# foxcroftjn/polars-strsim

Hardware: AMD Instinct MI355X
Metric: M string-pairs/s, levenshtein, 100 M rows (+ achieved HBM GB/s in roofline) (higher is better)
Workload: dtype u8/u32 bit-parallel, f64 epilogue

## Files before the change

polars-strsim_amd/csrc/strsim_lane_core.h:

```cpp
#pragma once
#include <stdint.h>
#include <type_traits>

#if defined(__HIPCC__)
#define STRSIM_HD __host__ __device__ __forceinline__
#else
#define STRSIM_HD inline
#endif

namespace strsim {

enum Measure : int { LEVENSHTEIN = 0, JARO = 1, JARO_WINKLER = 2, JACCARD = 3, SORENSEN_DICE = 4 };


#ifndef STRSIM_COLS_PER_TEST
#define STRSIM_COLS_PER_TEST 2
#endif
constexpr int COLS_PER_TEST = STRSIM_COLS_PER_TEST;

STRSIM_HD uint32_t lane_byte(const uint32_t (&w)[8], int j) { return (w[j >> 2] >> ((j & 3) * 8)) & 0xFFu; }

STRSIM_HD uint32_t low_ones(uint32_t k) { return k >= 32u ? 0xFFFFFFFFu : ((1u << k) - 1u); }

template <int G, int NG, typename F>
// ... 105 lines not shown
            r[4 * h + 1] = perm_b32(t2, t0, 0x07060302u);
            r[4 * h + 2] = perm_b32(t3, t1, 0x05040100u);
            r[4 * h + 3] = perm_b32(t3, t1, 0x07060302u);
        }
    }
#pragma unroll
    for (int e = 0; e < 8; e += 2) {
        const uint32_t a = r[e], b = r[e + 1];
        r[e] = bitop3<0xCA>(0x55555555u, a, twice(b));
        r[e + 1] = bitop3<0xCA>(0x55555555u, a >> 1, b);
    }
#pragma unroll
    for (int q = 0; q < 4; ++q) {
        const int e = (q & 1) | ((q & 2) << 1);
        const uint32_t a = r[e], b = r[e + 2];
        r[e] = bitop3<0xCA>(0x33333333u, a, b << 2);
        r[e + 2] = bitop3<0xCA>(0x33333333u, a >> 2, b);
    }
#pragma unroll
    for (int e = 0; e < 4; ++e) {
        const uint32_t a = r[e], b = r[e + 4];
        if (e < NP) P[e < NP ? e : 0] = bitop3<0xCA>(0x0F0F0F0Fu, a, b << 4);
        if (e + 4 < NP) P[e + 4 < NP ? e + 4 : 0] = bitop3<0xCA>(0x0F0F0F0Fu, a >> 4, b);
    }
}

template <int NP>
STRSIM_HD uint32_t eq_mask(const uint32_t (&P)[NP], uint32_t valid, uint32_t w, int byte)
{
    uint32_t acc = valid;
#pragma unroll
    for (int k = 0; k < NP; ++k) acc = bitop3<0x90>(acc, P[k], bit_fill(w, 8 * byte + k));
    return acc;
}

STRSIM_HD int planes_needed(uint32_t vary) { return (vary & 0x40u) ? 7 : ((vary & 0x20u) ? 6 : 5); }

STRSIM_HD uint32_t window_vary(const uint32_t (&wa)[8], const uint32_t (&wb)[8], uint32_t &any)
{
    uint32_t o = bitop3<0xFE>(wa[0], wa[1], wa[2]), n = bitop3<0x80>(wa[0], wa[1], wa[2]);
    o = bitop3<0xFE>(o, wa[3], wa[4]); n = bitop3<0x80>(n, wa[3], wa[4]);
    o = bitop3<0xFE>(o, wa[5], wa[6]); n = bitop3<0x80>(n, wa[5], wa[6]);
    o = bitop3<0xFE>(o, wa[7], wb[0]); n = bitop3<0x80>(n, wa[7], wb[0]);
    o = bitop3<0xFE>(o, wb[1], wb[2]); n = bitop3<0x80>(n, wb[1], wb[2]);
    o = bitop3<0xFE>(o, wb[3], wb[4]); n = bitop3<0x80>(n, wb[3], wb[4]);
    o = bitop3<0xFE>(o, wb[5], wb[6]); n = bitop3<0x80>(n, wb[5], wb[6]);
    o |= wb[7]; n &= wb[7];
    uint32_t o8 = o | (o >> 16); o8 |= o8 >> 8;
    uint32_t n8 = n & (n >> 16); n8 &= n8 >> 8;
    any = o8 & 0xFFu;
    return (o8 ^ n8) & 0xFFu;
}

template <int NP>
STRSIM_HD uint32_t lev_myers32_snap(const uint32_t (&wt)[8], uint32_t lt, uint32_t tmin, uint32_t tmax, const uint32_t (&P)[NP],
                                    uint32_t lp)
{
    uint32_t Pv = 0xFFFFFFFFu, Mv = 0u;
#pragma unroll
    for (int g = 0; g < 32 / COLS_PER_TEST; ++g) {
        if ((uint32_t)(COLS_PER_TEST * g) >= tmax) break;
        auto column = [&](int j) {
            const uint32_t Eq = eq_mask<NP>(P, 0xFFFFFFFFu, wt[j >> 2], j & 3);
            const uint32_t D0 = bitop3<0xBE>((Eq & Pv) + Pv, Pv, Eq) | Mv;
            const uint32_t nHP = bitop3<0x0E>(Mv, D0, Pv);
            const uint32_t nX = twice(nHP);
            const uint32_t HN2 = twice(D0 & Pv);
            Pv = bitop3<0xF2>(HN2, D0, nX);
            Mv = bitop3<0x50>(D0, D0, nX);
        };
        if ((uint32_t)(COLS_PER_TEST * (g + 1)) >= tmin) {
#pragma unroll
            for (int jj = 0; jj < COLS_PER_TEST; ++jj)
                if ((uint32_t)(COLS_PER_TEST * g + jj) < lt) column(COLS_PER_TEST * g + jj);
        } else {
#pragma unroll
            for (int jj = 0; jj < COLS_PER_TEST; ++jj) column(COLS_PER_TEST * g + jj);
        }
    }
    const uint32_t rows = low_ones(lp);
    return lt + popc32(Pv & rows) - popc32(Mv & rows);
}

STRSIM_HD uint32_t common_prefix4(uint32_t a0, uint32_t la, uint32_t b0, uint32_t lb)
{
    const uint32_t x = a0 ^ b0;
    uint32_t p = 4u;
    if (x & 0x000000FFu) p = 0u;
    else if (x & 0x0000FF00u) p = 1u;
    else if (x & 0x00FF0000u) p = 2u;
    else if (x & 0xFF000000u) p = 3u;
    if (p > la) p = la;
    if (p > lb) p = lb;
    return p;
}

STRSIM_HD double epilogue_levenshtein(uint64_t dist, uint64_t la, uint64_t lb)
{
    const uint64_t den = la > lb ? la : lb;
    return 1.0 - ((double)dist / (double)den);
}

STRSIM_HD double epilogue_jaro(uint64_t m, uint64_t t, uint64_t la, uint64_t lb)
{
    if (m == 0) return 0.0;
    const double dm = (double)m;
    return (dm / (double)la + dm / (double)lb + (double)(m - t / 2) / dm) / 3.0;
}

STRSIM_HD double epilogue_jaro_winkler(double jaro, uint32_t prefix)
{
    if (jaro > 0.7) {
        const double pl = (double)prefix;
        return jaro + (pl * 0.1 * (1.0 - jaro));
    }
    return jaro;
}

STRSIM_HD double epilogue_jaccard(uint64_t isect, uint64_t la, uint64_t lb)
{
    return (double)isect / (double)(la + lb - isect);
}

STRSIM_HD double epilogue_sorensen_dice(uint64_t isect, uint64_t la, uint64_t lb)
{
    return 2.0 * (double)isect / (double)(la + lb);
}
// ... 93 lines not shown
```

polars-strsim_amd/csrc/strsim_lane_stage.h:

```cpp
#pragma once

#ifndef STRSIM_STAGE_ROWS
#define STRSIM_STAGE_ROWS 512
#endif
#ifndef STRSIM_STAGE_CAP
#define STRSIM_STAGE_CAP 10240
#endif
#ifndef STRSIM_STAGE_CAP_LONG
#define STRSIM_STAGE_CAP_LONG 15104
#endif
#ifndef STRSIM_STAGE_CAP_LUT
#define STRSIM_STAGE_CAP_LUT 8960
#endif
#ifndef STRSIM_STAGE_WAVES_PER_EU
#define STRSIM_STAGE_WAVES_PER_EU 5
#endif
#ifndef STRSIM_STAGE_BUCKET_SHIFT
#define STRSIM_STAGE_BUCKET_SHIFT 1
#endif

#ifndef STRSIM_STAGE_LUT
#define STRSIM_STAGE_LUT 0x26
#endif
#ifndef STRSIM_JARO_KEEP_EQ_FILLS
#define STRSIM_JARO_KEEP_EQ_FILLS 1
#endif
#ifndef STRSIM_STAGE_LONG_TEXT_MAX
#define STRSIM_STAGE_LONG_TEXT_MAX 32
#endif
#ifndef STRSIM_STAGE_RANGE_MAX
#define STRSIM_STAGE_RANGE_MAX 64
#endif
#ifndef STRSIM_STAGE_RANGE_DIV
#define STRSIM_STAGE_RANGE_DIV 4
#endif
#ifndef STRSIM_STAGE_RANGE_MIN_BLOCKS
#define STRSIM_STAGE_RANGE_MIN_BLOCKS 2
#endif

#if defined(STRSIM_LAB) && defined(STRSIM_STAGE_STAMPS)
__device__ unsigned long long g_stage_stamps[16384][16];
#define STAGE_STAMP(cat) do { __builtin_amdgcn_sched_barrier(0); const unsigned long long t_ = __builtin_amdgcn_s_memtime(); \
                              __builtin_amdgcn_sched_barrier(0); st_acc[cat] += t_ - st_last; st_last = t_; } while (0)
#else
#define STAGE_STAMP(cat) do { } while (0)
#endif

#ifndef STRSIM_STAGE_THREADS
#define STRSIM_STAGE_THREADS 256
#endif
constexpr int STAGE_BLOCK = STRSIM_STAGE_THREADS;
constexpr int STAGE_WAVES = STAGE_BLOCK / 64;
constexpr int STAGE_ROWS = STRSIM_STAGE_ROWS;
constexpr int STAGE_RPT = STAGE_ROWS / STAGE_BLOCK;
constexpr int STAGE_NR = STAGE_ROWS / 64;
constexpr int STAGE_RPW = STAGE_NR / STAGE_WAVES;
template <int MEASURE> constexpr bool stage_uses_lut() { return ((STRSIM_STAGE_LUT >> MEASURE) & 1) != 0; }

template <bool TABLES, bool LONG = false> struct StageGeom {
    static_assert(!(TABLES && LONG), "the long-row geometry has no match-mask tables");
    static constexpr int CAP = LONG ? STRSIM_STAGE_CAP_LONG : (TABLES ? STRSIM_STAGE_CAP_LUT : STRSIM_STAGE_CAP);
    static constexpr int COL = CAP + 96;
    static constexpr int DMA_ITERS = (CAP + 48 + 16 * STAGE_BLOCK - 1) / (16 * STAGE_BLOCK);
    static_assert(CAP % 16 == 0 && 2 * COL + 64 + 16 <= 65536, "staging area: whole wave-instructions, 16-bit LDS offsets");
};
constexpr int STAGE_BSH = STRSIM_STAGE_BUCKET_SHIFT;
constexpr int STAGE_NBK = (32 >> STAGE_BSH) + 1;
static_assert(STAGE_RPT >= 1 && STAGE_RPT <= 4 && STAGE_RPW >= 1, "STAGE_ROWS is 256, 512 or 1024");
static_assert(STAGE_NBK <= 32, "the bucket scan runs on 32 lanes");

#define STRSIM_LDS_ADDR(p) ((uint32_t)(uintptr_t)((__attribute__((address_space(3))) void *)(p)))

__device__ __forceinline__ void lds_dma_b128(const void *gbase, uint32_t goff, uint32_t lds_dst)
{
    uint32_t keep;
    asm volatile("s_mov_b32 %0, m0\n\ts_mov_b32 m0, %3\n\ts_nop 0\n\tglobal_load_lds_dwordx4 %1, %2\n\ts_mov_b32 m0, %0"
                 : "=&s"(keep)
                 : "v"(goff), "s"(gbase), "s"(lds_dst)
                 : "memory");
}
__device__ __forceinline__ void lds_dma_b32(const void *gbase, uint32_t goff, uint32_t lds_dst)
{
    uint32_t keep;
    asm volatile("s_mov_b32 %0, m0\n\ts_mov_b32 m0, %3\n\ts_nop 0\n\tglobal_load_lds_dword %1, %2\n\ts_mov_b32 m0, %0"
                 : "=&s"(keep)
                 : "v"(goff), "s"(gbase), "s"(lds_dst)
                 : "memory");
}

__device__ __forceinline__ uint32_t load_invariant(const uint32_t *p)
{
    return *reinterpret_cast<const __attribute__((address_space(4))) uint32_t *>(reinterpret_cast<uintptr_t>(p));
}

constexpr uint32_t STAGE_DEAD = 1u << 31;

#if defined(STRSIM_LAB) && defined(STRSIM_STAGE_STRIP)
__device__ const uint16_t *g_strip_ptr;
__global__ __launch_bounds__(256) void k_strip_oracle(const uint32_t *__restrict__ offA, const uint8_t *__restrict__ valA, const uint32_t *__restrict__ offB,
                                                      const uint8_t *__restrict__ valB, uint64_t n, uint16_t *__restrict__ out)
{
    const uint64_t r = (uint64_t)blockIdx.x * 256u + threadIdx.x;
    if (r >= n) return;
    const uint32_t a0 = offA[r], la = offA[r + 1] - a0, b0 = offB[r], lb = offB[r + 1] - b0;
    const uint32_t m = la < lb ? la : lb, cap = (uint32_t)STRSIM_STAGE_STRIP;
    uint32_t p = 0, s = 0;
    while (p < m && p < cap && valA[a0 + p] == valB[b0 + p]) ++p;
    while (s < m - p && s < cap && valA[a0 + la - 1u - s] == valB[b0 + lb - 1u - s]) ++s;
    if (p + s > 63u) s = 63u - p;
    out[r] = (uint16_t)(p | (s << 8));
}
#define STRSIM_STRIP_ON 1
#else
#define STRSIM_STRIP_ON 0
#endif

__device__ __forceinline__ void stage_window(const uint8_t *base, uint32_t at, uint32_t (&w)[8], uint32_t lds_bytes = 0u, uint32_t who = 0u)
{
    typedef uint32_t u32x4_a4 __attribute__((ext_vector_type(4), aligned(4)));
    (void)lds_bytes; (void)who;
    if (who == 1u) STRSIM_CHECK_RANGE(K_STAGE, 40, ~0ull, (at & ~3u) + 36u, 0, lds_bytes);
    if (who == 2u) STRSIM_CHECK_RANGE(K_LIT, 40, ~0ull, (at & ~3u) + 36u, 0, lds_bytes);
    const uint8_t *q = base + (at & ~3u);
    const u32x4_a4 lo = *reinterpret_cast<const u32x4_a4 *>(q);
    const u32x4_a4 hi = *reinterpret_cast<const u32x4_a4 *>(q + 16);
    const uint32_t top = *reinterpret_cast<const uint32_t *>(q + 32);
    const uint32_t sh = at & 3u;
    w[0] = __builtin_amdgcn_alignbyte(lo.y, lo.x, sh); w[1] = __builtin_amdgcn_alignbyte(lo.z, lo.y, sh);
    w[2] = __builtin_amdgcn_alignbyte(lo.w, lo.z, sh); w[3] = __builtin_amdgcn_alignbyte(hi.x, lo.w, sh);
    w[4] = __builtin_amdgcn_alignbyte(hi.y, hi.x, sh); w[5] = __builtin_amdgcn_alignbyte(hi.z, hi.y, sh);
    w[6] = __builtin_amdgcn_alignbyte(hi.w, hi.z, sh); w[7] = __builtin_amdgcn_alignbyte(top, hi.w, sh);
}

__device__ __forceinline__ uint32_t scan32_inclusive(uint32_t x)
{
    x += (uint32_t)__builtin_amdgcn_update_dpp(0, (int)x, 0x111, 0xF, 0xF, true);
    x += (uint32_t)__builtin_amdgcn_update_dpp(0, (int)x, 0x112, 0xF, 0xF, true);
    x += (uint32_t)__builtin_amdgcn_update_dpp(0, (int)x, 0x114, 0xF, 0xF, true);
    x += (uint32_t)__builtin_amdgcn_update_dpp(0, (int)x, 0x118, 0xF, 0xF, true);
    x += (uint32_t)__builtin_amdgcn_update_dpp(0, (int)x, 0x142, 0xA, 0xF, true);
    return x;
}

template <int NP, bool USE_LUT>
__device__ __forceinline__ uint32_t stage_lev_code(const EqLut &lut, const uint32_t (&wa)[8], uint32_t la, const uint32_t (&wb)[8],
                                                   uint32_t lb, uint32_t tmin, uint32_t tmax, uint32_t stripped = 0u)
{
    uint32_t P[NP];
    build_planes<NP>(wb, P);
    EqLut t = lut;
    if (USE_LUT) lut_build<NP>(t, P, 0xFFFFFFFFu);
    const bool live = la != 0u && lb != 0u;
    const uint32_t la1 = live ? la : 1u, lb1 = live ? lb : 1u;
    const uint32_t dist = USE_LUT ? lev_myers32_lut<NP>(t, wa, la1, tmin, tmax, P, lb1) : lev_myers32_snap<NP>(wa, la1, tmin, tmax, P, lb1);
    uint32_t code = dist * (uint32_t)QTAB_N + (la1 > lb1 ? la1 : lb1);
    if (!live) code = (la == 0u && lb == 0u) ? 1u : (uint32_t)QTAB_N + 1u;
#if STRSIM_STRIP_ON
    const uint32_t longer = la > lb ? la : lb;
    code = (live ? dist : longer) * (uint32_t)QTAB_N + (longer + stripped);
#endif
    return code;
}

template <int NP, bool USE_LUT>
__device__ __forceinline__ unsigned long long stage_all_ints(const EqLut &lut, const uint32_t (&wa)[8], uint32_t la,
                                                             const uint32_t (&wb)[8], uint32_t lb, uint32_t tmin, uint32_t tmax)
{
    uint32_t P[NP];
    build_planes<NP>(wb, P);
    const bool live = la != 0u && lb != 0u;
    const uint32_t la1 = live ? la : 1u, lb1 = live ? lb : 1u;
    uint32_t dist, m, t, isect;
    if (USE_LUT) {
        EqLut tb = lut;
        lut_build<NP>(tb, P, 0xFFFFFFFFu);
        lane_cores32_lut<NP, true, true, true>(tb, wa, la1, tmin, tmax, lb1, P, dist, m, t, isect);
    } else {
        lane_cores32<NP, true, true, true>(wa, la1, tmin, tmax, lb1, P, dist, m, t, isect);
    }
    const uint32_t pre = common_prefix4(wa[0], la1, wb[0], lb1);
    const uint32_t lo = dist | (m << 6) | (t << 12) | (isect << 18) | (pre << 24) | (la << 27);
    return (unsigned long long)lo | ((unsigned long long)(la >> 5) << 32) | ((unsigned long long)lb << 33);
}

__device__ __forceinline__ void stage_all_epilogues(unsigned long long pk, double qa, double qb, double qc, double qd, double (&r)[5])
{
    const uint32_t lo = (uint32_t)pk, hi = (uint32_t)(pk >> 32);
    const uint32_t m = (lo >> 6) & 63u, isect = (lo >> 18) & 63u, pre = (lo >> 24) & 7u;
    const uint32_t la = ((lo >> 27) & 31u) | ((hi & 1u) << 5), lb = (hi >> 1) & 63u;
    if (la == 0u || lb == 0u) {
        const double v = (la == 0u && lb == 0u) ? 1.0 : 0.0;
#pragma unroll
        for (int q = 0; q < 5; ++q) r[q] = v;
        return;
    }
    r[LEVENSHTEIN] = 1.0 - qd;
    const double j = m == 0u ? 0.0 : div3_exact(qa + qb + qc);
    r[JARO] = j;
    r[JARO_WINKLER] = epilogue_jaro_winkler(j, pre);
    r[JACCARD] = epilogue_jaccard(isect, la, lb);
    r[SORENSEN_DICE] = epilogue_sorensen_dice(isect, la, lb);
}

template <int MEASURE, int NP, bool USE_LUT>
__device__ __forceinline__ uint32_t stage_ints(const EqLut &lut, const uint32_t (&wa)[8], uint32_t la, const uint32_t (&wb)[8],
                                               uint32_t lb, uint32_t tmin, uint32_t tmax)
{
    uint32_t P[NP];
    build_planes<NP>(wb, P);
    const bool live = la != 0u && lb != 0u;
    const uint32_t la1 = live ? la : 1u, lb1 = live ? lb : 1u;
    uint32_t dist, m, t, isect;
    EqLut tb = lut;
    if (USE_LUT) lut_build<NP>(tb, P, 0xFFFFFFFFu);
    if (MEASURE == JARO || MEASURE == JARO_WINKLER) {
        if (USE_LUT) lane_cores32_lut<NP, false, true, false>(tb, wa, la1, tmin, tmax, lb1, P, dist, m, t, isect);
        else lane_cores32<NP, false, true, false, STRSIM_JARO_KEEP_EQ_FILLS != 0>(wa, la1, tmin, tmax, lb1, P, dist, m, t, isect);
        const uint32_t pre = MEASURE == JARO_WINKLER ? common_prefix4(wa[0], la1, wb[0], lb1) : 0u;
        return m | (t << 6) | (la << 12) | (lb << 18) | (pre << 24);
    }
    if (USE_LUT) lane_cores32_lut<NP, false, false, true>(tb, wa, la1, tmin, tmax, lb1, P, dist, m, t, isect);
    else lane_cores32<NP, false, false, true>(wa, la1, tmin, tmax, lb1, P, dist, m, t, isect);
    return isect | (la << 6) | (lb << 12);
}

template <int MEASURE>
__device__ __forceinline__ double stage_epilogue(uint32_t pk, double qa, double qb, double qc)
{
    if (MEASURE == JARO || MEASURE == JARO_WINKLER) {
        const uint32_t m = pk & 63u, la = (pk >> 12) & 63u, lb = (pk >> 18) & 63u, pre = (pk >> 24) & 7u;
        if (la == 0u || lb == 0u) return (la == 0u && lb == 0u) ? 1.0 : 0.0;
        const double j = m == 0u ? 0.0 : div3_exact(qa + qb + qc);
        return MEASURE == JARO_WINKLER ? epilogue_jaro_winkler(j, pre) : j;
    }
    const uint32_t isect = pk & 63u, la = (pk >> 6) & 63u, lb = (pk >> 12) & 63u;
    if (la == 0u || lb == 0u) return (la == 0u && lb == 0u) ? 1.0 : 0.0;
    return MEASURE == JACCARD ? epilogue_jaccard(isect, la, lb) : epilogue_sorensen_dice(isect, la, lb);
}

template <int MEASURE, bool LUT>
__device__ __forceinline__ void stage_compute(const EqLut &lut, const uint32_t (&wt)[8], const uint32_t (&wp)[8], uint32_t meta,
                                              uint32_t last, uint16_t *s_code, uint32_t *s_word, double *s_val)
{
    bool fast = (meta & STAGE_DEAD) == 0u;
#if STRSIM_STRIP_ON
    const uint32_t lt = meta & 0x3Fu, lp = (meta >> 8) & 0x3Fu, idx = (meta >> 16) & 0x1FFu, stripped = (meta >> 25) & 0x3Fu;
#else
    const uint32_t lt = meta & 0x3Fu, lp = (meta >> 8) & 0x3Fu, idx = (meta >> 16) & 0x7FFu, stripped = 0u;
#endif
    uint32_t any;
    const uint32_t vary = window_vary(wt, wp, any);
    if (any & 0x80u) fast = false;
    if (__ballot(fast) == 0ull) return;
    const uint32_t la = fast ? lt : 0u, lb = fast ? lp : 0u;
    static_assert((1 << STAGE_BSH) % COLS_PER_TEST == 0, "a bucket's upper bound is a whole number of column groups");
    const uint32_t ltl = (uint32_t)__builtin_amdgcn_readlane((int)lt, (int)last);
    const uint32_t tmax = (((ltl ? ltl : 1u) - 1u) | ((1u << STAGE_BSH) - 1u)) + 1u;
    const bool wide = __ballot(fast && (vary & 0x60u)) != 0ull;
    const uint32_t lt0 = uniform(lt);
    const uint32_t tmin = (((lt0 ? lt0 : 1u) - 1u) & ~((1u << STAGE_BSH) - 1u)) + 1u;
    if (MEASURE == LEVENSHTEIN) {
        uint32_t code;
        if (wide) code = stage_lev_code<7, LUT>(lut, wt, la, wp, lb, tmin, tmax, stripped);
        else code = stage_lev_code<5, LUT>(lut, wt, la, wp, lb, tmin, tmax, stripped);
        if (fast) STRSIM_CHECK_INDEX(K_STAGE, 42, ~0ull, idx, STAGE_ROWS);
        if (fast) s_code[idx] = (uint16_t)code;
    } else if (MEASURE == ALL_MEASURES) {
        unsigned long long pk;
        if (wide) pk = stage_all_ints<7, LUT>(lut, wt, la, wp, lb, tmin, tmax);
        else pk = stage_all_ints<5, LUT>(lut, wt, la, wp, lb, tmin, tmax);
        if (fast) STRSIM_CHECK_INDEX(K_STAGE, 43, ~0ull, idx, STAGE_ROWS);
        if (fast) reinterpret_cast<unsigned long long *>(s_val)[idx] = pk;
    } else {
        uint32_t pk;
        if (wide) pk = stage_ints<MEASURE, 7, LUT>(lut, wt, la, wp, lb, tmin, tmax);
        else pk = stage_ints<MEASURE, 5, LUT>(lut, wt, la, wp, lb, tmin, tmax);
        if (fast) STRSIM_CHECK_INDEX(K_STAGE, 44, ~0ull, idx, STAGE_ROWS);
        if (fast) s_word[idx] = pk;
    }
}

template <int MEASURE, bool LUT, bool LONG = false>
__device__ __forceinline__ void
lane_stage_body(const uint32_t *__restrict__ offA, const uint8_t *__restrict__ valA, uint64_t rowsA,
             const uint32_t *__restrict__ offB, const uint8_t *__restrict__ valB, uint64_t rowsB, OutPtrs outs,
             uint64_t n, unsigned long long *__restrict__ slowmask, DevStatus *__restrict__ status,
             const double *__restrict__ qtab, uint32_t *__restrict__ sched, DevStatus *__restrict__ publish, uint32_t ticket)
{
    constexpr bool LEV = MEASURE == LEVENSHTEIN;
    constexpr bool ALL = MEASURE == ALL_MEASURES;
    constexpr int B = STAGE_ROWS, RPT = STAGE_RPT, NBK = STAGE_NBK;
    constexpr int STAGE_CAP = StageGeom<LUT, LONG>::CAP, STAGE_COL = StageGeom<LUT, LONG>::COL;
    constexpr int STAGE_DMA_ITERS = StageGeom<LUT, LONG>::DMA_ITERS;
    constexpr uint32_t COLB = STAGE_COL, LIT = 2u * STAGE_COL;
    static_assert(!LUT || (B <= 128 * STAGE_WAVES && LUT_WAVE_BYTES == 3072), "descriptor slices: 128 rows behind each wave's tables");
    __shared__ __attribute__((aligned(4096))) uint8_t s_lut[LUT ? 4096 * STAGE_WAVES : 16];
    __shared__ uint2 s_desc_own[LUT ? 1 : B];
    __shared__ __attribute__((aligned(4096))) uint8_t s_bytes[2 * STAGE_COL + 64 + 16];
    auto desc_at = [&](uint32_t p) -> uint2 * {
        if (LUT) return reinterpret_cast<uint2 *>(s_lut + ((p >> 7) << 12) + LUT_WAVE_BYTES + ((p & 127u) << 3));
        return s_desc_own + p;
    };
    __shared__ __attribute__((aligned(16))) uint32_t s_off[2][B + 4];
    __shared__ uint32_t s_cnt[32];
    __shared__ uint32_t s_left;
    __shared__ uint32_t s_sched[2];
    __shared__ uint16_t s_code[LEV ? B : 1];
    __shared__ uint32_t s_word[(!LEV && !ALL) ? B : 1];
    __shared__ double s_val[ALL ? B : 1];

    const uint32_t tid = threadIdx.x, lane = lane_id(), wv = tid >> 6;
    if (blockIdx.x == 0u && tid < (uint32_t)(sizeof(DevStatus) / sizeof(uint32_t))) reinterpret_cast<uint32_t *>(status)[tid] = 0u;
    if (tid < 32u) s_cnt[tid] = 0u;
    if (tid == 0u) s_left = 0u;
#pragma unroll
    for (int q = 0; q < RPT; ++q) {
        const uint32_t i = (uint32_t)q * STAGE_BLOCK + tid;
        if (LEV) s_code[i] = 0xFFFFu;
        else if (ALL) reinterpret_cast<unsigned long long *>(&s_val[i])[0] = ~0ull;
        else s_word[i] = 0xFFFFFFFFu;
    }

    const uint32_t totalA = load_invariant(offA + rowsA), totalB = load_invariant(offB + rowsB);
#if STRSIM_BOUNDS_ON
    const uint32_t firstA = load_invariant(offA), firstB = load_invariant(offB);
#endif
    const bool bcastA = rowsA == 1, bcastB = rowsB == 1;
    const uint32_t litA0 = bcastA ? load_invariant(offA) : 0u, litB0 = bcastB ? load_invariant(offB) : 0u;
    const uint32_t litAlen = bcastA ? totalA - litA0 : 0u, litBlen = bcastB ? totalB - litB0 : 0u;
    if (wv == 0u) {
        auto literal_window = [&](const uint8_t *val, uint32_t at, uint32_t total, uint32_t len, uint32_t *dst) {
            uint32_t w[8];
            load_window32(val, at, total, w);
            const uint32_t rep = (w[0] & 0xFFu) * 0x01010101u;
#pragma unroll
            for (int q = 0; q < 8; ++q) {
                const uint32_t v = len > 4u * q ? (len - 4u * q < 4u ? len - 4u * q : 4u) : 0u;
                const uint32_t keep = v >= 4u ? 0xFFFFFFFFu : ((1u << (8u * v)) - 1u);
                dst[q] = (w[q] & keep) | (rep & ~keep);
            }
        };
        if (bcastA) literal_window(valA, litA0, totalA, litAlen, reinterpret_cast<uint32_t *>(s_bytes + LIT));
        if (bcastB) literal_window(valB, litB0, totalB, litBlen, reinterpret_cast<uint32_t *>(s_bytes + LIT + 32u));
    }
    const uint64_t nchunks = (n + 63u) >> 6;
    const uint32_t nchunks32 = (uint32_t)nchunks;
    auto grab = [&](uint32_t seen, uint32_t &lo, uint32_t &sz) {
        const uint32_t left = nchunks32 > seen ? nchunks32 - seen : 0u;
        uint32_t want = (uint32_t)STRSIM_STAGE_RANGE_MAX;
        if (left < (uint32_t)(STRSIM_STAGE_RANGE_MAX * STRSIM_STAGE_RANGE_DIV) * gridDim.x) want = left / ((uint32_t)STRSIM_STAGE_RANGE_DIV * gridDim.x);
        sz = want < (uint32_t)(STRSIM_STAGE_RANGE_MIN_BLOCKS * (B / 64)) ? (uint32_t)(STRSIM_STAGE_RANGE_MIN_BLOCKS * (B / 64)) : want;
        lo = __hip_atomic_fetch_add(&sched[0], sz, __ATOMIC_RELAXED, __HIP_MEMORY_SCOPE_AGENT);
    };
    uint32_t grab_lo = 0u, grab_sz = 0u;
    if (tid == 0u) {
        grab(0u, grab_lo, grab_sz);
        s_sched[0] = grab_lo;
        s_sched[1] = grab_sz;
    }
    lds_barrier();
    uint64_t row_end;
    uint64_t row0;
    {
        const uint64_t lo = uniform(s_sched[0]), hi = lo + uniform(s_sched[1]);
        row0 = lo * 64u < n ? lo * 64u : n;
        row_end = hi * 64u < n ? hi * 64u : n;
    }
// ... 84 lines not shown
            if (JARO_LIKE) { pin(t1[q]); pin(t2[q]); }
            if (ALL) pin(t3[q]);
        }
#pragma unroll
        for (int q = 0; q < RPT; ++q) {
            const uint32_t i = (uint32_t)q * STAGE_BLOCK + tid;
            if ((uint32_t)q * STAGE_BLOCK < rows) {
                bool undone;
                double v = 0.0, v5[5];
                if (ALL) {
                    undone = pk[q] == ~0ull;
                    if (!undone) stage_all_epilogues(pk[q], t0[q], t1[q], t2[q], t3[q], v5);
                } else if (LEV) {
                    undone = (uint32_t)pk[q] == 0xFFFFu;
                    v = 1.0 - t0[q];
                } else {
                    undone = (uint32_t)pk[q] == 0xFFFFFFFFu;
                    if (!undone) v = stage_epilogue<M1>((uint32_t)pk[q], t0[q], t1[q], t2[q]);
                }
                const bool valid = i < rows;
                const unsigned long long left = __ballot(undone && valid);
                if (valid) STRSIM_CHECK_INDEX(K_STAGE, 10, r0 + i, r0 + i, n);
                if (lane == 0u && valid) STRSIM_CHECK_INDEX(K_STAGE, 11, r0 + i, (r0 >> 6) + (i >> 6), nchunks);
                if (valid && !undone) {
                    if (ALL) {
#pragma unroll
                        for (int o = 0; o < 5; ++o) outs.p[o][r0 + i] = v5[o];
                    } else {
                        outs.p[0][r0 + i] = v;
                    }
                }
                if (lane == 0u && valid) {
                    maskb[i >> 6] = left;
                    if (publish && left) atomicAdd(&s_left, (uint32_t)__builtin_popcountll(left));
                }
            }
        }
    };

#if defined(STRSIM_LAB) && defined(STRSIM_STAGE_STAMPS)
    unsigned long long st_acc[10] = {0, 0, 0, 0, 0, 0, 0, 0, 0, 0};
    const unsigned long long st_t0 = __builtin_amdgcn_s_memtime(), st_r0 = __builtin_amdgcn_s_memrealtime();
    unsigned long long st_last = st_t0;
#endif
    while (row0 < row_end) {
        if (grab_pending) {
            if (tid == 0u) {
                s_sched[0] = grab_lo;
                s_sched[1] = grab_sz;
            }
            grab_pending = false;
        }
        if (prev_rows) store_block(prev_row0, prev_rows);
        STAGE_STAMP(1);
        const uint32_t avail = (uint32_t)(row_end - row0 < (uint64_t)B ? row_end - row0 : (uint64_t)B);
        const uint32_t baseA = bcastA ? litA0 : uniform(s_off[0][0]), baseB = bcastB ? litB0 : uniform(s_off[1][0]);
        const uint32_t misA = (uint32_t)(reinterpret_cast<uintptr_t>(valA + baseA) & 15u);
        const uint32_t misB = (uint32_t)(reinterpret_cast<uintptr_t>(valB + baseB) & 15u);
        uint32_t rows;
        {
            const uint32_t e = (lane + 1u) * 64u < avail ? (lane + 1u) * 64u : avail;
            const bool exists = lane * 64u < avail && lane < (uint32_t)(B / 64);
            const uint32_t endA = bcastA ? baseA : s_off[0][exists ? e : 0u], endB = bcastB ? baseB : s_off[1][exists ? e : 0u];
            const bool fits = exists && endA - baseA + misA <= (uint32_t)STAGE_CAP && endB - baseB + misB <= (uint32_t)STAGE_CAP;
            const unsigned long long okm = __ballot(fits);
            uint32_t k = (uint32_t)__builtin_ctzll(~okm);
            if (k == 0u) k = 1u;
            rows = uniform(k * 64u < avail ? k * 64u : avail);
        }
        const uint32_t endA = bcastA ? baseA : uniform(s_off[0][rows]), endB = bcastB ? baseB : uniform(s_off[1][rows]);
        const uint32_t spanA = endA - baseA + misA, spanB = endB - baseB + misB;
        const uint32_t stagedA = bcastA ? 0u : (((spanA < (uint32_t)STAGE_CAP ? spanA : (uint32_t)STAGE_CAP) + 15u) & ~15u);
        const uint32_t stagedB = bcastB ? 0u : (((spanB < (uint32_t)STAGE_CAP ? spanB : (uint32_t)STAGE_CAP) + 15u) & ~15u);
        const uint32_t leftA = totalA - baseA + misA, leftB = totalB - baseB + misB;
        const uint32_t chunksA = bcastA ? 0u : ((stagedA + 32u < leftA ? stagedA + 32u : leftA) + 15u) >> 4;
        const uint32_t chunksB = bcastB ? 0u : ((stagedB + 32u < leftB ? stagedB + 32u : leftB) + 15u) >> 4;
        if (tid < 2u) STRSIM_CHECK_RANGE(K_STAGE, 20, row0, (chunksA << 4) + tid * 16u + 16u, 0, COLB);
        else if (tid < 4u) STRSIM_CHECK_RANGE(K_STAGE, 21, row0, COLB + (chunksB << 4) + (tid - 2u) * 16u + 16u, 0, sizeof(s_bytes));
        if (tid < 2u) *reinterpret_cast<uint4 *>(s_bytes + (chunksA << 4) + tid * 16u) = make_uint4(0u, 0u, 0u, 0u);
        else if (tid < 4u) *reinterpret_cast<uint4 *>(s_bytes + COLB + (chunksB << 4) + (tid - 2u) * 16u) = make_uint4(0u, 0u, 0u, 0u);
        {
            const uint8_t *__restrict__ const gA = valA + baseA - misA, *__restrict__ const gB = valB + baseB - misB;
#pragma unroll
            for (int it = 0; it < STAGE_DMA_ITERS; ++it) {
                if (tid + (uint32_t)it * STAGE_BLOCK < chunksA) {
                    STRSIM_CHECK_COLUMN(K_STAGE, 22, row0, gA + 16 * it * STAGE_BLOCK + tid16, 16, valA, firstA, totalA);
                    STRSIM_CHECK_RANGE(K_STAGE, 23, row0, 16u * ((uint32_t)it * STAGE_BLOCK + tid) + 16u, 0, COLB);
                    lds_dma_b128(gA + 16 * it * STAGE_BLOCK, tid16, ldsBytes + 16u * ((uint32_t)it * STAGE_BLOCK + wvu * 64u));
                }
                if (tid + (uint32_t)it * STAGE_BLOCK < chunksB) {
                    STRSIM_CHECK_COLUMN(K_STAGE, 24, row0, gB + 16 * it * STAGE_BLOCK + tid16, 16, valB, firstB, totalB);
                    STRSIM_CHECK_RANGE(K_STAGE, 25, row0, COLB + 16u * ((uint32_t)it * STAGE_BLOCK + tid) + 16u, 0, sizeof(s_bytes));
                    lds_dma_b128(gB + 16 * it * STAGE_BLOCK, tid16, ldsBytes + COLB + 16u * ((uint32_t)it * STAGE_BLOCK + wvu * 64u));
                }
            }
        }
        STAGE_STAMP(0);
        uint32_t skey[RPT], srank[RPT], sd0[RPT], sd1[RPT];
        {
#pragma unroll
            for (int q = 0; q < RPT; ++q) {
                const uint32_t i = (uint32_t)RPT * tid + (uint32_t)q;
                STRSIM_CHECK_INDEX(K_STAGE, 30, row0, i + 1u, B + 4);
                const bool have = i < rows;
                const uint32_t a0 = bcastA ? 0u : s_off[0][i] - baseA, b0 = bcastB ? 0u : s_off[1][i] - baseB;
                const uint32_t la8 = bcastA ? litAlen : s_off[0][i + 1u] - s_off[0][i];
                const uint32_t lb8 = bcastB ? litBlen : s_off[1][i + 1u] - s_off[1][i];
                const bool stA = bcastA || misA + a0 + la8 <= stagedA, stB = bcastB || misB + b0 + lb8 <= stagedB;
                bool mine = have && la8 <= 32u && lb8 <= 32u && stA && stB;
                if (LONG && STRSIM_STAGE_LONG_TEXT_MAX < 32 && !bcastA && !bcastB) mine = mine && (la8 < lb8 ? la8 : lb8) <= (uint32_t)STRSIM_STAGE_LONG_TEXT_MAX;
                const uint32_t wa = bcastA ? LIT : misA + a0, wb = bcastB ? LIT + 32u : COLB + misB + b0;
                const bool swap = !bcastA && !bcastB && la8 > lb8;
#if STRSIM_STRIP_ON
                uint32_t sp = 0u, ss = 0u;
                if (LEV && !bcastA && !bcastB && have) {
                    const uint32_t ps = g_strip_ptr[row0 + i];
                    sp = ps & 0xFFu; ss = ps >> 8;
                }
                const uint32_t lt = (swap ? lb8 : la8) - sp - ss, lp = (swap ? la8 : lb8) - sp - ss;
                const uint32_t key = mine ? (((lt ? lt : 1u) - 1u) >> STAGE_BSH) : (uint32_t)(NBK - 1);
                skey[q] = key;
                srank[q] = atomicAdd(&s_cnt[key], 1u);
                sd0[q] = mine ? (swap ? ((wb + sp) | ((wa + sp) << 16)) : ((wa + sp) | ((wb + sp) << 16))) : 0u;
                sd1[q] = mine ? (lt | (lp << 8) | (i << 16) | ((sp + ss) << 25)) : STAGE_DEAD;
#else
                const uint32_t lt = swap ? lb8 : la8, lp = swap ? la8 : lb8;
                const uint32_t key = mine ? (((lt ? lt : 1u) - 1u) >> STAGE_BSH) : (uint32_t)(NBK - 1);
                skey[q] = key;
                srank[q] = atomicAdd(&s_cnt[key], 1u);
                sd0[q] = mine ? (swap ? (wb | (wa << 16)) : (wa | (wb << 16))) : 0u;
                sd1[q] = mine ? (lt | (lp << 8) | (i << 16)) : STAGE_DEAD;
#endif
            }
        }
        STAGE_STAMP(2);
        lds_barrier();
        STAGE_STAMP(3);
        uint32_t nmine;
        {
            const uint32_t c = s_cnt[lane & 31u];
            const uint32_t exc = scan32_inclusive(c) - c;
#pragma unroll
            for (int q = 0; q < RPT; ++q) {
                const uint32_t base = __shfl(exc, skey[q], 32);
                const uint32_t p = base + srank[q];
                STRSIM_CHECK_INDEX(K_STAGE, 31, row0, p, B);
                *desc_at(p) = make_uint2(sd0[q], sd1[q]);
            }
            nmine = uniform(__shfl(exc, NBK - 1, 32));
        }
        STAGE_STAMP(4);
        asm volatile("s_waitcnt vmcnt(0)" ::: "memory");
        if (!bcastA && leftA < (chunksA << 4) && tid == ((chunksA - 1u) & (uint32_t)(STAGE_BLOCK - 1)))
            for (uint32_t b = leftA; b < (chunksA << 4); ++b) { STRSIM_CHECK_INDEX(K_STAGE, 32, row0, b, COLB); s_bytes[b] = 0; }
        if (!bcastB && leftB < (chunksB << 4) && tid == ((chunksB - 1u) & (uint32_t)(STAGE_BLOCK - 1)))
            for (uint32_t b = leftB; b < (chunksB << 4); ++b) { STRSIM_CHECK_INDEX(K_STAGE, 33, row0, COLB + b, sizeof(s_bytes)); s_bytes[COLB + b] = 0; }
        lds_barrier();
        STAGE_STAMP(5);
        if (tid < 32u) s_cnt[tid] = 0u;
        uint64_t next_row0 = row0 + rows;
        if (next_row0 >= row_end) {
            const uint64_t lo = uniform(s_sched[0]), hi = lo + uniform(s_sched[1]);
            next_row0 = lo * 64u < n ? lo * 64u : n;
            row_end = hi * 64u < n ? hi * 64u : n;
            if (tid == 0u) grab((uint32_t)lo, grab_lo, grab_sz);
            grab_pending = true;
        }
        if (next_row0 < row_end) dma_offsets(next_row0);
        STAGE_STAMP(6);
        __builtin_amdgcn_s_setprio(0);
        {
            const uint32_t nrounds = (nmine + 63u) >> 6;
#pragma unroll 1
            for (int k = 0; k < STAGE_RPW; ++k) {
                const uint32_t t = (uint32_t)(k >> 1) * (2u * STAGE_WAVES) + ((k & 1) ? (uint32_t)(2 * STAGE_WAVES - 1) - wv : wv);
                if (t >= nrounds) continue;
                const uint32_t hi = nmine - 64u * t;
                const uint32_t first = hi >= 64u ? hi - 64u : 0u;
                const uint32_t in_round = hi - first;
                __builtin_amdgcn_s_setprio(1);
                STRSIM_CHECK_INDEX(K_STAGE, 41, row0, first + lane, B);
                const uint2 d = *desc_at(first + lane);
                uint32_t wt[8], wp[8];
                stage_window(s_bytes, d.x & 0xFFFFu, wt, (uint32_t)sizeof(s_bytes), STRSIM_BOUNDS_ON ? 1u : 0u);
                stage_window(s_bytes, d.x >> 16, wp, (uint32_t)sizeof(s_bytes), STRSIM_BOUNDS_ON ? 1u : 0u);
    #if defined(STRSIM_LAB) && defined(STRSIM_STAGE_STAMPS)
                asm volatile("s_waitcnt lgkmcnt(0)" ::: "memory");
    #endif
                STAGE_STAMP(7);
                __builtin_amdgcn_s_setprio(0);
                stage_compute<MEASURE, LUT>(lut, wt, wp, lane < in_round ? d.y : STAGE_DEAD, in_round - 1u, s_code, s_word, s_val);
                STAGE_STAMP(8);
            }
        }
        __builtin_amdgcn_s_setprio(1);
        asm volatile("s_waitcnt vmcnt(0)" ::: "memory");
        lds_barrier();
        STAGE_STAMP(9);
        prev_row0 = row0;
        prev_rows = rows;
        row0 = next_row0;
    }
    if (prev_rows) store_block(prev_row0, prev_rows);
    if (publish) lds_barrier();
    if (tid == 0u) {
        if (publish && s_left) __hip_atomic_fetch_add(&sched[2], s_left, __ATOMIC_RELAXED, __HIP_MEMORY_SCOPE_AGENT);
        const uint32_t done = __hip_atomic_fetch_add(&sched[1], 1u, __ATOMIC_ACQ_REL, __HIP_MEMORY_SCOPE_AGENT);
        if (done == gridDim.x - 1u) {
            if (publish) {
                const uint32_t total = __hip_atomic_load(&sched[2], __ATOMIC_RELAXED, __HIP_MEMORY_SCOPE_AGENT);
                __hip_atomic_store(&publish->lane_left, total, __ATOMIC_RELEASE, __HIP_MEMORY_SCOPE_SYSTEM);
                if (ticket) __hip_atomic_store(&publish->ticket, ticket, __ATOMIC_RELEASE, __HIP_MEMORY_SCOPE_SYSTEM);
            }
            __hip_atomic_store(&sched[0], 0u, __ATOMIC_RELAXED, __HIP_MEMORY_SCOPE_AGENT);
            __hip_atomic_store(&sched[1], 0u, __ATOMIC_RELAXED, __HIP_MEMORY_SCOPE_AGENT);
            __hip_atomic_store(&sched[2], 0u, __ATOMIC_RELAXED, __HIP_MEMORY_SCOPE_AGENT);
        }
    }
#if defined(STRSIM_LAB) && defined(STRSIM_STAGE_STAMPS)
    if (lane == 0u) {
        const uint32_t w = (blockIdx.x * STAGE_WAVES + wv) & 16383u;
        for (int q = 0; q < 10; ++q) g_stage_stamps[w][q] = st_acc[q];
        g_stage_stamps[w][10] = __builtin_amdgcn_s_memtime() - st_t0;
        const unsigned long long st_r1 = __builtin_amdgcn_s_memrealtime();
        g_stage_stamps[w][11] = st_r1 - st_r0;
        g_stage_stamps[w][12] = st_r0;
        g_stage_stamps[w][13] = st_r1;
        g_stage_stamps[w][14] = (unsigned long long)__builtin_amdgcn_s_getreg((4 << 0) | (0 << 6) | (31 << 11));
        g_stage_stamps[w][15] = (unsigned long long)__builtin_amdgcn_s_getreg((20 << 0) | (0 << 6) | (31 << 11));
    }
#endif
}

#ifndef STRSIM_STAGE_PLAIN_WAVES
#define STRSIM_STAGE_PLAIN_WAVES 5
#endif
#ifndef STRSIM_STAGE_ALL_WAVES_PER_EU
#define STRSIM_STAGE_ALL_WAVES_PER_EU 3
#endif
template <int MEASURE, bool TABLES, bool LONG = false> constexpr int stage_waves_per_eu()
{
    constexpr int lim = MEASURE == ALL_MEASURES ? STRSIM_STAGE_ALL_WAVES_PER_EU : ((TABLES || LONG) ? 4 : STRSIM_STAGE_PLAIN_WAVES);
    return STRSIM_STAGE_WAVES_PER_EU < lim ? STRSIM_STAGE_WAVES_PER_EU : lim;
}
// ... 20 lines not shown
```

polars-strsim_amd/csrc/strsim_lane_stage_pc.h:

```cpp
#pragma once

#ifndef STRSIM_PC_CAP
#define STRSIM_PC_CAP 10240
#endif
#ifndef STRSIM_PC_WG_PER_CU
#define STRSIM_PC_WG_PER_CU 2
#endif
#ifndef STRSIM_PC_LUT
#define STRSIM_PC_LUT 1
#endif

constexpr int PC_THREADS = 512, PC_PROD = 256, PC_CW = 4;

template <int MEASURE, bool LUT>
__device__ __forceinline__ void
lane_stage_pc_body(const uint32_t *__restrict__ offA, const uint8_t *__restrict__ valA, uint64_t rowsA,
                   const uint32_t *__restrict__ offB, const uint8_t *__restrict__ valB, uint64_t rowsB, OutPtrs outs,
                   uint64_t n, unsigned long long *__restrict__ slowmask, DevStatus *__restrict__ status,
                   const double *__restrict__ qtab, uint32_t *__restrict__ sched, DevStatus *__restrict__ publish, uint32_t ticket)
{
    static_assert(MEASURE != ALL_MEASURES, "single measures only");
    constexpr bool LEV = MEASURE == LEVENSHTEIN;
    constexpr int B = STAGE_ROWS, RPT = B / PC_PROD, NBK = STAGE_NBK;
    constexpr int CAP = STRSIM_PC_CAP, COL = CAP + 96, AREA = 2 * COL + 64 + 16;
    constexpr int DMA_ITERS = (CAP + 48 + 16 * PC_PROD - 1) / (16 * PC_PROD);
    constexpr uint32_t COLB = COL;
    static_assert(B == 512 && RPT == 2 && B / 64 == 2 * PC_CW, "eight rounds per block, two per consumer wave");
    static_assert(CAP % 16 == 0 && AREA <= 65536 && AREA % 16 == 0, "staging area");

    __shared__ __attribute__((aligned(4096))) uint8_t s_lut[LUT ? 4096 * PC_CW : 16];
    __shared__ __attribute__((aligned(16))) uint8_t s_bytes[2][AREA];
    __shared__ uint2 s_desc[2][B];
    __shared__ __attribute__((aligned(16))) uint32_t s_off[2][B + 4];
    __shared__ uint32_t s_cnt[2][32];
    __shared__ uint32_t s_rows[2], s_nmine[2];
    __shared__ uint32_t s_left, s_sched[2];
    __shared__ uint16_t s_code[2][LEV ? B : 1];
    __shared__ uint32_t s_word[2][LEV ? 1 : B];
    __shared__ double s_none[1];

    const uint32_t tid = threadIdx.x, lane = lane_id(), wv = tid >> 6;
    const bool producer = uniform(wv) < 4u;
    const uint32_t ptid = tid & (uint32_t)(PC_PROD - 1);
    const uint32_t pwv = uniform(wv & 3u);
    if (blockIdx.x == 0u && tid < (uint32_t)(sizeof(DevStatus) / sizeof(uint32_t))) reinterpret_cast<uint32_t *>(status)[tid] = 0u;
    if (tid < 64u) s_cnt[tid >> 5][tid & 31u] = 0u;
    if (tid == 0u) { s_left = 0u; s_rows[0] = s_rows[1] = 0u; s_nmine[0] = s_nmine[1] = 0u; }
    if (producer) {
#pragma unroll
        for (int q = 0; q < 2 * RPT; ++q) {
            const uint32_t i = (uint32_t)q * PC_PROD + ptid;
            if (LEV) s_code[i / B][i % B] = 0xFFFFu;
            else s_word[i / B][i % B] = 0xFFFFFFFFu;
        }
    }
    const uint32_t totalA = load_invariant(offA + rowsA), totalB = load_invariant(offB + rowsB);

    const uint64_t nchunks = (n + 63u) >> 6;
    const uint32_t nchunks32 = (uint32_t)nchunks;
    auto grab = [&](uint32_t seen, uint32_t &lo, uint32_t &sz) {
        const uint32_t left = nchunks32 > seen ? nchunks32 - seen : 0u;
        uint32_t want = (uint32_t)STRSIM_STAGE_RANGE_MAX;
        if (left < (uint32_t)(STRSIM_STAGE_RANGE_MAX * STRSIM_STAGE_RANGE_DIV) * gridDim.x) want = left / ((uint32_t)STRSIM_STAGE_RANGE_DIV * gridDim.x);
        sz = want < (uint32_t)(STRSIM_STAGE_RANGE_MIN_BLOCKS * (B / 64)) ? (uint32_t)(STRSIM_STAGE_RANGE_MIN_BLOCKS * (B / 64)) : want;
        lo = __hip_atomic_fetch_add(&sched[0], sz, __ATOMIC_RELAXED, __HIP_MEMORY_SCOPE_AGENT);
    };
    uint32_t grab_lo = 0u, grab_sz = 0u;
    if (tid == 0u) {
        grab(0u, grab_lo, grab_sz);
        s_sched[0] = grab_lo;
        s_sched[1] = grab_sz;
    }
    lds_barrier();
    uint64_t row_end, row0;
    {
        const uint64_t lo = uniform(s_sched[0]), hi = lo + uniform(s_sched[1]);
// ... 281 lines not shown
```

Baseline: 70990.

## Sort rows by exact text length and load narrow text windows

Bucket shift now defaults to 0, so rows are sorted into 33 exact-length buckets instead of length pairs. The bucket prefix scan widens to a full 64-lane wave. With exact buckets, the Myers column loop stops at the true maximum text length instead of a rounded column group. Rounds whose longest text fits in 16 bytes load a 20-byte LDS window instead of 36 bytes. An optional block-wide character-class precomputation (off by default) is added, and the producer/consumer variant now statically requires the old bucket shift, which could break that build form under the new default.

```diff
diff --git a/polars-strsim_amd/csrc/strsim_lane_core.h b/polars-strsim_amd/csrc/strsim_lane_core.h
--- a/polars-strsim_amd/csrc/strsim_lane_core.h
+++ b/polars-strsim_amd/csrc/strsim_lane_core.h
@@ -181,7 +181,7 @@
     return (o8 ^ n8) & 0xFFu;
 }
 
-template <int NP>
+template <int NP, bool EXACT = false>
 STRSIM_HD uint32_t lev_myers32_snap(const uint32_t (&wt)[8], uint32_t lt, uint32_t tmin, uint32_t tmax, const uint32_t (&P)[NP],
                                     uint32_t lp)
 {
@@ -200,8 +200,10 @@
         };
         if ((uint32_t)(COLS_PER_TEST * (g + 1)) >= tmin) {
 #pragma unroll
-            for (int jj = 0; jj < COLS_PER_TEST; ++jj)
+            for (int jj = 0; jj < COLS_PER_TEST; ++jj) {
+                if (EXACT && jj > 0 && (uint32_t)(COLS_PER_TEST * g + jj) >= tmax) break;
                 if ((uint32_t)(COLS_PER_TEST * g + jj) < lt) column(COLS_PER_TEST * g + jj);
+            }
         } else {
 #pragma unroll
             for (int jj = 0; jj < COLS_PER_TEST; ++jj) column(COLS_PER_TEST * g + jj);
diff --git a/polars-strsim_amd/csrc/strsim_lane_stage.h b/polars-strsim_amd/csrc/strsim_lane_stage.h
--- a/polars-strsim_amd/csrc/strsim_lane_stage.h
+++ b/polars-strsim_amd/csrc/strsim_lane_stage.h
@@ -16,7 +16,13 @@
 #define STRSIM_STAGE_WAVES_PER_EU 5
 #endif
 #ifndef STRSIM_STAGE_BUCKET_SHIFT
-#define STRSIM_STAGE_BUCKET_SHIFT 1
+#define STRSIM_STAGE_BUCKET_SHIFT 0
+#endif
+#ifndef STRSIM_STAGE_BLOCK_CLASS
+#define STRSIM_STAGE_BLOCK_CLASS 0
+#endif
+#ifndef STRSIM_STAGE_NARROW_TEXT
+#define STRSIM_STAGE_NARROW_TEXT 1
 #endif
 
 #ifndef STRSIM_STAGE_LUT
@@ -67,7 +73,7 @@
 constexpr int STAGE_BSH = STRSIM_STAGE_BUCKET_SHIFT;
 constexpr int STAGE_NBK = (32 >> STAGE_BSH) + 1;
 static_assert(STAGE_RPT >= 1 && STAGE_RPT <= 4 && STAGE_RPW >= 1, "STAGE_ROWS is 256, 512 or 1024");
-static_assert(STAGE_NBK <= 32, "the bucket scan runs on 32 lanes");
+static_assert(STAGE_NBK <= 64, "the bucket scan runs on one wave");
 
 #define STRSIM_LDS_ADDR(p) ((uint32_t)(uintptr_t)((__attribute__((address_space(3))) void *)(p)))
 
@@ -132,6 +138,20 @@
     w[6] = __builtin_amdgcn_alignbyte(hi.w, hi.z, sh); w[7] = __builtin_amdgcn_alignbyte(top, hi.w, sh);
 }
 
+__device__ __forceinline__ void stage_window16(const uint8_t *base, uint32_t at, uint32_t (&w)[8], uint32_t lds_bytes = 0u, uint32_t who = 0u)
+{
+    typedef uint32_t u32x4_a4 __attribute__((ext_vector_type(4), aligned(4)));
+    (void)lds_bytes; (void)who;
+    if (who == 1u) STRSIM_CHECK_RANGE(K_STAGE, 40, ~0ull, (at & ~3u) + 20u, 0, lds_bytes);
+    const uint8_t *q = base + (at & ~3u);
+    const u32x4_a4 lo = *reinterpret_cast<const u32x4_a4 *>(q);
+    const uint32_t top = *reinterpret_cast<const uint32_t *>(q + 16);
+    const uint32_t sh = at & 3u;
+    w[0] = __builtin_amdgcn_alignbyte(lo.y, lo.x, sh); w[1] = __builtin_amdgcn_alignbyte(lo.z, lo.y, sh);
+    w[2] = __builtin_amdgcn_alignbyte(lo.w, lo.z, sh); w[3] = __builtin_amdgcn_alignbyte(top, lo.w, sh);
+    w[4] = w[3]; w[5] = w[3]; w[6] = w[3]; w[7] = w[3];
+}
+
 __device__ __forceinline__ uint32_t scan32_inclusive(uint32_t x)
 {
     x += (uint32_t)__builtin_amdgcn_update_dpp(0, (int)x, 0x111, 0xF, 0xF, true);
@@ -142,6 +162,32 @@
     return x;
 }
 
+__device__ __forceinline__ uint32_t scan64_inclusive(uint32_t x, uint32_t lane)
+{
+    x = scan32_inclusive(x);
+    const uint32_t low = (uint32_t)__builtin_amdgcn_readlane((int)x, 31);
+    return lane >= 32u ? x + low : x;
+}
+
+constexpr uint32_t STAGE_CLS_HIGH = 0x80u;
+__device__ __forceinline__ uint32_t stage_class_vary(uint32_t cls) { return cls & (cls >> 8) & 0x60u; }
+
+__device__ __forceinline__ void class_chunk_masked(const uint4 v, uint32_t at, uint32_t lo, uint32_t hi, uint32_t &o, uint32_t &n)
+{
+    const uint32_t d[4] = {v.x, v.y, v.z, v.w};
+#pragma unroll
+    for (int q = 0; q < 4; ++q) {
+        const int b = (int)at + 4 * q;
+        const int s = (int)lo - b, e = (int)hi - b;
+        const int s4 = s < 0 ? 0 : (s > 4 ? 4 : s), e4 = e < 0 ? 0 : (e > 4 ? 4 : e);
+        const uint32_t below_e = e4 >= 4 ? 0xFFFFFFFFu : ((1u << (8 * e4)) - 1u);
+        const uint32_t below_s = s4 >= 4 ? 0xFFFFFFFFu : ((1u << (8 * s4)) - 1u);
+        const uint32_t keep = below_e & ~below_s;
+        o |= d[q] & keep;
+        n &= d[q] | ~keep;
+    }
+}
+
 template <int NP, bool USE_LUT>
 __device__ __forceinline__ uint32_t stage_lev_code(const EqLut &lut, const uint32_t (&wa)[8], uint32_t la, const uint32_t (&wb)[8],
                                                    uint32_t lb, uint32_t tmin, uint32_t tmax, uint32_t stripped = 0u)
@@ -152,7 +198,7 @@
     if (USE_LUT) lut_build<NP>(t, P, 0xFFFFFFFFu);
     const bool live = la != 0u && lb != 0u;
     const uint32_t la1 = live ? la : 1u, lb1 = live ? lb : 1u;
-    const uint32_t dist = USE_LUT ? lev_myers32_lut<NP>(t, wa, la1, tmin, tmax, P, lb1) : lev_myers32_snap<NP>(wa, la1, tmin, tmax, P, lb1);
+    const uint32_t dist = USE_LUT ? lev_myers32_lut<NP>(t, wa, la1, tmin, tmax, P, lb1) : lev_myers32_snap<NP, STAGE_BSH == 0>(wa, la1, tmin, tmax, P, lb1);
     uint32_t code = dist * (uint32_t)QTAB_N + (la1 > lb1 ? la1 : lb1);
     if (!live) code = (la == 0u && lb == 0u) ? 1u : (uint32_t)QTAB_N + 1u;
 #if STRSIM_STRIP_ON
@@ -240,7 +286,8 @@
 
 template <int MEASURE, bool LUT>
 __device__ __forceinline__ void stage_compute(const EqLut &lut, const uint32_t (&wt)[8], const uint32_t (&wp)[8], uint32_t meta,
-                                              uint32_t last, uint16_t *s_code, uint32_t *s_word, double *s_val)
+                                              uint32_t last, uint16_t *s_code, uint32_t *s_word, double *s_val,
+                                              uint32_t cls = STAGE_CLS_HIGH)
 {
     bool fast = (meta & STAGE_DEAD) == 0u;
 #if STRSIM_STRIP_ON
@@ -248,15 +295,19 @@
 #else
     const uint32_t lt = meta & 0x3Fu, lp = (meta >> 8) & 0x3Fu, idx = (meta >> 16) & 0x7FFu, stripped = 0u;
 #endif
-    uint32_t any;
-    const uint32_t vary = window_vary(wt, wp, any);
-    if (any & 0x80u) fast = false;
+    const bool per_round = (cls & STAGE_CLS_HIGH) != 0u;
+    uint32_t vary = stage_class_vary(cls);
+    if (per_round) {
+        uint32_t any;
+        vary = window_vary(wt, wp, any);
+        if (any & 0x80u) fast = false;
+    }
     if (__ballot(fast) == 0ull) return;
     const uint32_t la = fast ? lt : 0u, lb = fast ? lp : 0u;
-    static_assert((1 << STAGE_BSH) % COLS_PER_TEST == 0, "a bucket's upper bound is a whole number of column groups");
+    static_assert(STAGE_BSH == 0 || (1 << STAGE_BSH) % COLS_PER_TEST == 0, "a bucket's upper bound is a whole number of column groups");
     const uint32_t ltl = (uint32_t)__builtin_amdgcn_readlane((int)lt, (int)last);
     const uint32_t tmax = (((ltl ? ltl : 1u) - 1u) | ((1u << STAGE_BSH) - 1u)) + 1u;
-    const bool wide = __ballot(fast && (vary & 0x60u)) != 0ull;
+    const bool wide = per_round ? __ballot(fast && (vary & 0x60u)) != 0ull : vary != 0u;
     const uint32_t lt0 = uniform(lt);
     const uint32_t tmin = (((lt0 ? lt0 : 1u) - 1u) & ~((1u << STAGE_BSH) - 1u)) + 1u;
     if (MEASURE == LEVENSHTEIN) {
@@ -302,7 +353,8 @@
         return s_desc_own + p;
     };
     __shared__ __attribute__((aligned(16))) uint32_t s_off[2][B + 4];
-    __shared__ uint32_t s_cnt[32];
+    __shared__ uint32_t s_cnt[NBK];
+    __shared__ uint32_t s_cls;
     __shared__ uint32_t s_left;
     __shared__ uint32_t s_sched[2];
     __shared__ uint16_t s_code[LEV ? B : 1];
@@ -311,8 +363,9 @@
 
     const uint32_t tid = threadIdx.x, lane = lane_id(), wv = tid >> 6;
     if (blockIdx.x == 0u && tid < (uint32_t)(sizeof(DevStatus) / sizeof(uint32_t))) reinterpret_cast<uint32_t *>(status)[tid] = 0u;
-    if (tid < 32u) s_cnt[tid] = 0u;
+    if (tid < (uint32_t)NBK) s_cnt[tid] = 0u;
     if (tid == 0u) s_left = 0u;
+    if (tid == 0u) s_cls = 0u;
 #pragma unroll
     for (int q = 0; q < RPT; ++q) {
         const uint32_t i = (uint32_t)q * STAGE_BLOCK + tid;
@@ -503,6 +556,7 @@
             grab_pending = false;
         }
         if (prev_rows) store_block(prev_row0, prev_rows);
+        if (tid == 0u) s_cls = 0u;
         STAGE_STAMP(1);
         const uint32_t avail = (uint32_t)(row_end - row0 < (uint64_t)B ? row_end - row0 : (uint64_t)B);
         const uint32_t baseA = bcastA ? litA0 : uniform(s_off[0][0]), baseB = bcastB ? litB0 : uniform(s_off[1][0]);
@@ -589,26 +643,60 @@
         STAGE_STAMP(3);
         uint32_t nmine;
         {
-            const uint32_t c = s_cnt[lane & 31u];
-            const uint32_t exc = scan32_inclusive(c) - c;
+            const uint32_t c = lane < (uint32_t)NBK ? s_cnt[lane] : 0u;
+            const uint32_t exc = (NBK <= 32 ? scan32_inclusive(c) : scan64_inclusive(c, lane)) - c;
 #pragma unroll
             for (int q = 0; q < RPT; ++q) {
-                const uint32_t base = __shfl(exc, skey[q], 32);
+                const uint32_t base = __shfl(exc, skey[q], 64);
                 const uint32_t p = base + srank[q];
                 STRSIM_CHECK_INDEX(K_STAGE, 31, row0, p, B);
                 *desc_at(p) = make_uint2(sd0[q], sd1[q]);
             }
-            nmine = uniform(__shfl(exc, NBK - 1, 32));
+            nmine = uniform((uint32_t)__builtin_amdgcn_readlane((int)exc, NBK - 1));
         }
         STAGE_STAMP(4);
         asm volatile("s_waitcnt vmcnt(0)" ::: "memory");
+#if STRSIM_STAGE_BLOCK_CLASS
+        if (!bcastA && !bcastB) {
+            uint32_t o = 0u, nn = 0xFFFFFFFFu;
+            auto column = [&](uint32_t col, uint32_t lo, uint32_t hi) {
+                const uint32_t nch = (hi + 15u) >> 4;
+                if (hi <= lo) return;
+#pragma unroll
+                for (int it = 0; it < STAGE_DMA_ITERS; ++it) {
+                    const uint32_t c = (uint32_t)it * STAGE_BLOCK + tid;
+                    if (c - 1u < nch - 2u && nch >= 2u) {
+                        STRSIM_CHECK_RANGE(K_STAGE, 26, row0, col + 16u * c + 16u, 0, sizeof(s_bytes));
+                        const uint4 v = *reinterpret_cast<const uint4 *>(s_bytes + col + 16u * c);
+                        o = bitop3<0xFE>(o, v.x, v.y); o = bitop3<0xFE>(o, v.z, v.w);
+                        nn = bitop3<0x80>(nn, v.x, v.y); nn = bitop3<0x80>(nn, v.z, v.w);
+                    }
+                }
+                auto edge = [&](uint32_t c) {
+                    STRSIM_CHECK_RANGE(K_STAGE, 27, row0, col + 16u * c + 16u, 0, sizeof(s_bytes));
+                    const uint4 v = *reinterpret_cast<const uint4 *>(s_bytes + col + 16u * c);
+                    class_chunk_masked(v, 16u * c, lo, hi, o, nn);
+                };
+                if (tid == 0u) edge(0u);
+                if (nch >= 2u && tid == ((nch - 1u) & (uint32_t)(STAGE_BLOCK - 1))) edge(nch - 1u);
+            };
+            column(0u, misA, spanA < stagedA ? spanA : stagedA);
+            column(COLB, misB, spanB < stagedB ? spanB : stagedB);
+            uint32_t o8 = o | (o >> 16); o8 |= o8 >> 8;
+            uint32_t n8 = nn & (nn >> 16); n8 &= n8 >> 8;
+            const uint32_t wcls = (__ballot((o8 & 0x80u) != 0u) ? 0x80u : 0u) | (__ballot((o8 & 0x40u) != 0u) ? 0x40u : 0u) |
+                                  (__ballot((o8 & 0x20u) != 0u) ? 0x20u : 0u) | (__ballot((n8 & 0x40u) == 0u) ? 0x4000u : 0u) |
+                                  (__ballot((n8 & 0x20u) == 0u) ? 0x2000u : 0u);
+            if (lane == 0u && wcls) atomicOr(&s_cls, wave_uniform(wcls));
+        }
+#endif
         if (!bcastA && leftA < (chunksA << 4) && tid == ((chunksA - 1u) & (uint32_t)(STAGE_BLOCK - 1)))
             for (uint32_t b = leftA; b < (chunksA << 4); ++b) { STRSIM_CHECK_INDEX(K_STAGE, 32, row0, b, COLB); s_bytes[b] = 0; }
         if (!bcastB && leftB < (chunksB << 4) && tid == ((chunksB - 1u) & (uint32_t)(STAGE_BLOCK - 1)))
             for (uint32_t b = leftB; b < (chunksB << 4); ++b) { STRSIM_CHECK_INDEX(K_STAGE, 33, row0, COLB + b, sizeof(s_bytes)); s_bytes[COLB + b] = 0; }
         lds_barrier();
         STAGE_STAMP(5);
-        if (tid < 32u) s_cnt[tid] = 0u;
+        if (tid < (uint32_t)NBK) s_cnt[tid] = 0u;
         uint64_t next_row0 = row0 + rows;
         if (next_row0 >= row_end) {
             const uint64_t lo = uniform(s_sched[0]), hi = lo + uniform(s_sched[1]);
@@ -622,6 +710,7 @@
         __builtin_amdgcn_s_setprio(0);
         {
             const uint32_t nrounds = (nmine + 63u) >> 6;
+            const uint32_t cls = (STRSIM_STAGE_BLOCK_CLASS && !bcastA && !bcastB) ? uniform(s_cls) : STAGE_CLS_HIGH;
 #pragma unroll 1
             for (int k = 0; k < STAGE_RPW; ++k) {
                 const uint32_t t = (uint32_t)(k >> 1) * (2u * STAGE_WAVES) + ((k & 1) ? (uint32_t)(2 * STAGE_WAVES - 1) - wv : wv);
@@ -633,14 +722,16 @@
                 STRSIM_CHECK_INDEX(K_STAGE, 41, row0, first + lane, B);
                 const uint2 d = *desc_at(first + lane);
                 uint32_t wt[8], wp[8];
-                stage_window(s_bytes, d.x & 0xFFFFu, wt, (uint32_t)sizeof(s_bytes), STRSIM_BOUNDS_ON ? 1u : 0u);
+                const uint32_t ltl = (uint32_t)__builtin_amdgcn_readlane((int)(d.y & 0x3Fu), (int)(in_round - 1u));
+                if (STRSIM_STAGE_NARROW_TEXT && ltl <= 16u) stage_window16(s_bytes, d.x & 0xFFFFu, wt, (uint32_t)sizeof(s_bytes), STRSIM_BOUNDS_ON ? 1u : 0u);
+                else stage_window(s_bytes, d.x & 0xFFFFu, wt, (uint32_t)sizeof(s_bytes), STRSIM_BOUNDS_ON ? 1u : 0u);
                 stage_window(s_bytes, d.x >> 16, wp, (uint32_t)sizeof(s_bytes), STRSIM_BOUNDS_ON ? 1u : 0u);
     #if defined(STRSIM_LAB) && defined(STRSIM_STAGE_STAMPS)
                 asm volatile("s_waitcnt lgkmcnt(0)" ::: "memory");
     #endif
                 STAGE_STAMP(7);
                 __builtin_amdgcn_s_setprio(0);
-                stage_compute<MEASURE, LUT>(lut, wt, wp, lane < in_round ? d.y : STAGE_DEAD, in_round - 1u, s_code, s_word, s_val);
+                stage_compute<MEASURE, LUT>(lut, wt, wp, lane < in_round ? d.y : STAGE_DEAD, in_round - 1u, s_code, s_word, s_val, cls);
                 STAGE_STAMP(8);
             }
         }
diff --git a/polars-strsim_amd/csrc/strsim_lane_stage_pc.h b/polars-strsim_amd/csrc/strsim_lane_stage_pc.h
--- a/polars-strsim_amd/csrc/strsim_lane_stage_pc.h
+++ b/polars-strsim_amd/csrc/strsim_lane_stage_pc.h
@@ -22,6 +22,7 @@
     static_assert(MEASURE != ALL_MEASURES, "single measures only");
     constexpr bool LEV = MEASURE == LEVENSHTEIN;
     constexpr int B = STAGE_ROWS, RPT = B / PC_PROD, NBK = STAGE_NBK;
+    static_assert(NBK <= 32, "this form scans 32 counters: build it with STRSIM_STAGE_BUCKET_SHIFT=1");
     constexpr int CAP = STRSIM_PC_CAP, COL = CAP + 96, AREA = 2 * COL + 64 + 16;
     constexpr int DMA_ITERS = (CAP + 48 + 16 * PC_PROD - 1) / (16 * PC_PROD);
     constexpr uint32_t COLB = COL;
```

After: 71660 (median of 6 runs). About the same (+0.9%).
